# xmindflow/cenet

Hardware: AMD Instinct MI355X
Metric: training images/sec (224x224, 4-class) (higher is better)
Workload: dtype bf16

## Files before the change

cenet_amd/csrc/conv_direct.hip:

```cpp
#include "common.h"
#include "../../include/cenet_hip.h"

#define TH 8
#define TW 32
typedef bf16_t bf;

__device__ __forceinline__ unsigned cd_f2bf(float f) { return cenet_f2bf(f); }

struct ConvDirectArgs {
  const bf16_t* x;
  const float* w;
  bf16_t* y;
  int B, H, W, dgrad, tiles_x, tiles_y, ntiles;
};

template <int CIN, int COUT, int KS, int NW>
__global__ __launch_bounds__(64 * NW, (CIN == 64 && COUT == 64) ? 1 : 2) void conv_direct_bf16_kernel(ConvDirectArgs a) {
  constexpr int NT = 64 * NW, RPW = TH / NW, NI = 2 * RPW;
  constexpr int CQ = CIN / 8, HH = TH + KS - 1, HW_ = TW + KS - 1, KK = KS * KS, PADK = KS / 2;
  constexpr int UNITS = CQ * HH * HW_;
  constexpr int UPT = (UNITS + NT - 1) / NT;
  constexpr int MT = COUT / 16;
  __shared__ __attribute__((aligned(16))) bf Ws[KK * CQ * COUT * 8];
  __shared__ __attribute__((aligned(16))) bf Xs[UNITS * 8];
  const int tid = threadIdx.x, wave = tid >> 6, lane = tid & 63, fr = lane & 15, fq = lane >> 4;

  for (int e = tid; e < KK * CIN * COUT; e += NT) {
    const int t = e % KK, rest = e / KK;
    int co, ci;
    float v;
    if (!a.dgrad) {
      ci = rest % CIN;
      co = rest / CIN;
      v = a.w[e];
    } else {
      co = rest % COUT;
      ci = rest / COUT;
      v = a.w[(long)(ci * COUT + co) * KK + (KK - 1 - t)];
    }
    Ws[((t * CQ + (ci >> 3)) * COUT + co) * 8 + (ci & 7)] = (bf)cd_f2bf(v);
// ... 30 lines not shown
      const int s = tid + NT * u;
      if (s < UNITS) {
        unsigned pk[4];
#pragma unroll
        for (int j = 0; j < 4; ++j) pk[j] = pre[u][2 * j] | (pre[u][2 * j + 1] << 16);
        memcpy(&Xs[s * 8], pk, 16);
      }
    }
  };

  const int G = gridDim.x < 8 ? (int)gridDim.x : 8;
  const int xcd = blockIdx.x % G, nloc = ((int)gridDim.x + G - 1 - xcd) / G;
  const int per = (a.ntiles + G - 1) / G;
  const int t_end = (xcd + 1) * per < a.ntiles ? (xcd + 1) * per : a.ntiles;
  int tile = xcd * per + (int)blockIdx.x / G;
  if (tile < t_end) load_halo(tile);
  for (; tile < t_end; tile += nloc) {
    __syncthreads();
    store_halo();
    __syncthreads();
    const int nxt = tile + nloc;
    if (nxt < t_end) load_halo(nxt);

    f32x4 acc[MT][NI];
#pragma unroll
    for (int mi = 0; mi < MT; ++mi)
#pragma unroll
      for (int ni = 0; ni < NI; ++ni) acc[mi][ni] = f32x4{0.f, 0.f, 0.f, 0.f};
#pragma unroll
    for (int t = 0; t < KK; ++t) {
// ... 5 lines not shown
#pragma unroll
        for (int mi = 0; mi < MT; ++mi) memcpy(&wf[mi], &Ws[((t * CQ + kb * 4 + fq) * COUT + mi * 16 + fr) * 8], 16);
#pragma unroll
        for (int ni = 0; ni < NI; ++ni) {
          const int row = RPW * wave + (ni >> 1), xs = 16 * (ni & 1);
          bf16x8 xf;
          memcpy(&xf, &Xs[(((kb * 4 + fq) * HH + row + ky) * HW_ + xs + fr + kx) * 8], 16);
#pragma unroll
          for (int mi = 0; mi < MT; ++mi) acc[mi][ni] = __builtin_amdgcn_mfma_f32_16x16x32_bf16(xf, wf[mi], acc[mi][ni], 0, 0, 0);
        }
      }
    }
    const int b = tile / (a.tiles_x * a.tiles_y), tt = tile - b * (a.tiles_x * a.tiles_y);
    const int ty = tt / a.tiles_x, tx = tt - ty * a.tiles_x;
    bf16_t* yb = a.y + (long)b * COUT * HWp;
#pragma unroll
    for (int ni = 0; ni < NI; ++ni) {
      const int oy = ty * TH + RPW * wave + (ni >> 1), ox = tx * TW + 16 * (ni & 1) + 4 * fq;
      if (oy < a.H && ox < a.W) {
#pragma unroll
        for (int mi = 0; mi < MT; ++mi) {
          bf16_t* dst = yb + (long)(mi * 16 + fr) * HWp + (long)oy * a.W + ox;
          if (ox + 3 < a.W && (a.W & 3) == 0) {
            float v[4] = {acc[mi][ni][0], acc[mi][ni][1], acc[mi][ni][2], acc[mi][ni][3]};
            st4v(dst, v);
          } else {
#pragma unroll
            for (int r = 0; r < 4; ++r)
              if (ox + r < a.W) stf(dst + r, acc[mi][ni][r]);
          }
        }
      }
    }
  }
}

extern "C" int cenet_conv_direct_supported(int Cin, int Cout, int k, int stride, int pad) {
  if (stride != 1 || pad != k / 2) return 0;
  if (k == 5 && Cin == 32 && Cout == 32) return 1;
  if (k == 3 && Cin == 64 && (Cout == 64 || Cout == 32)) return 1;
  if (k == 3 && Cin == 32 && Cout == 64) return 1;
  return 0;
}

extern "C" int cenet_conv_direct_bf16(const bf16_t* x, const float* w, bf16_t* y, int B, int Cin, int Cout, int H, int W, int k,
                                      int dgrad, hipStream_t stream) {
  if (!x || !w || !y || B <= 0 || H <= 0 || W <= 0) return CENET_EINVAL;
  if (((uintptr_t)y & 7) != 0) return CENET_EINVAL;
  if (!cenet_conv_direct_supported(Cin, Cout, k, 1, k / 2)) return CENET_EUNSUPPORTED;
  ConvDirectArgs a;
  a.x = x; a.w = w; a.y = y; a.B = B; a.H = H; a.W = W; a.dgrad = dgrad;
  a.tiles_x = cdiv(W, TW);
  a.tiles_y = cdiv(H, TH);
  a.ntiles = B * a.tiles_x * a.tiles_y;
  const bool two = !(k == 3 && Cin == 64 && Cout == 64);
  const int slots = two ? 512 : 256;
  int grid = a.ntiles < slots ? a.ntiles : slots;
  if (k == 5 && Cin == 32 && Cout == 32) {
    CENET_LAUNCH((conv_direct_bf16_kernel<32, 32, 5, 4>), dim3(grid), dim3(256), stream, a);
  } else if (k == 3 && Cin == 64 && Cout == 64) {
    CENET_LAUNCH((conv_direct_bf16_kernel<64, 64, 3, 8>), dim3(grid), dim3(512), stream, a);
  } else if (k == 3 && Cin == 64 && Cout == 32) {
    CENET_LAUNCH((conv_direct_bf16_kernel<64, 32, 3, 8>), dim3(grid), dim3(512), stream, a);
  } else {
    CENET_LAUNCH((conv_direct_bf16_kernel<32, 64, 3, 4>), dim3(grid), dim3(256), stream, a);
  }
  CENET_CHECK_LAUNCH();
  return CENET_OK;
}

struct ConvWgradArgs {
  const bf16_t* x;
  const bf16_t* dy;
  float* ws;
  int B, H, W, tiles_x, tiles_y, ntiles;
  int vec;
};

__device__ __forceinline__ unsigned funnel16(unsigned lo, unsigned hi) { return (lo >> 16) | (hi << 16); }

template <int V>
// ... 264 lines not shown
```

cenet_amd/csrc/norm.hip:

```cpp
#include "common.h"
#include <cstdlib>
#include "../../include/cenet_hip.h"

template <typename T>
__global__ __launch_bounds__(256) void layernorm_fwd_kernel(const T* __restrict__ x, const float* __restrict__ gamma,
                                                           const float* __restrict__ beta, T* __restrict__ y,
                                                           float* __restrict__ mean, float* __restrict__ rstd, int rows,
                                                           int C, float eps) {
  const int wave = threadIdx.x >> 6, lane = threadIdx.x & 63;
  const long row = (long)blockIdx.x * 4 + wave;
  if (row >= rows) return;
  const T* xr = x + row * C;
  float s = 0.f;
  for (int c = lane; c < C; c += 64) s += ldf(xr + c);
  const float mu = wave_sum(s) / C;
  float v = 0.f;
  for (int c = lane; c < C; c += 64) {
    float d = ldf(xr + c) - mu;
    v += d * d;
  }
  const float rs = rsqrtf(wave_sum(v) / C + eps);
  T* yr = y + row * C;
  for (int c = lane; c < C; c += 64) stf(yr + c, (ldf(xr + c) - mu) * rs * gamma[c] + beta[c]);
  if (lane == 0) {
// ... 1381 lines not shown
  BnFin fin;
  fin.S = bn_partial_launch<T>(x, sxb, B, C, HW, ws, stream);
  fin.ws = ws; fin.n = (float)((long)B * HW); fin.mean = mean; fin.var = var; fin.rmean = running_mean; fin.rvar = running_var;
  fin.momentum = momentum; fin.nbt = num_batches_tracked; fin.nbt_n = nbt_count;
  return bn_apply_launch<T>(x, sxb, y, syb, mean, var, eps, gamma, beta, act, slope, B, C, HW, fin, stream);
}
CENET_TWIN(bn_train_fwd, (const T* x, long sxb, T* y, long syb, float* ws, float* mean, float* var, float* running_mean,
                          float* running_var, float momentum, long* num_batches_tracked, float eps, const float* gamma,
                          const float* beta, int act, float slope, int B, int C, int HW, int nbt_count, hipStream_t stream),
           (x, sxb, y, syb, ws, mean, var, running_mean, running_var, momentum, num_batches_tracked, eps, gamma, beta, act, slope, B,
            C, HW, nbt_count, stream))
CENET_TWIN(bn_apply, (const T* x, long sxb, T* y, long syb, const float* mean, const float* var, float eps, const float* gamma,
                      const float* beta, int act, float slope, int B, int C, int HW, hipStream_t stream),
           (x, sxb, y, syb, mean, var, eps, gamma, beta, act, slope, B, C, HW, stream))

template <typename T>
static int bn_bwd_acc_impl(const T* dy, long sgb, const T* x, long sxb, T* dx, long sdb, const float* mean, const float* var,
                           float eps, const float* gamma, const float* beta, int act, float slope, int B, int C, int HW,
                           float* ws, float* dgamma_acc, float* dbeta_acc, hipStream_t stream, const T* dx_add = nullptr,
                           long sab = 0) {
  if (B <= 0 || C <= 0 || HW <= 0) return CENET_EINVAL;
  const long total = (long)B * HW;
  if (sizeof(T) == 2 && total <= 256 * BN1K_EPT) {
    CENET_LAUNCH(bn_bwd_1k_kernel, dim3(C), dim3(256), stream, (const bf16_t*)dy, sgb, (const bf16_t*)x, sxb, (bf16_t*)dx, sdb, mean,
                 var, eps, gamma, beta, act, slope, B, HW, dgamma_acc, dbeta_acc, (const bf16_t*)dx_add, sab);
    CENET_CHECK_LAUNCH();
    return CENET_OK;
  }
  if (bn_flat_ok<T>(C, HW, sgb, sxb, sdb) && (!dx_add || sab == (long)C * HW)) {
    const bool v4 = bn_v4_ok<T>(HW, dy, sgb, x, sxb, dx, sdb) && bn_v4_ok<T>(HW, dx_add, sab, x, sxb, dx, sdb);
// ... 57 lines not shown
```

cenet_amd/kern.py:

```python
from __future__ import annotations

import ctypes as C
import math
from typing import Optional

import torch

from . import _lib
from ._lib import EpiT, MatT

ACT = {"none": 0, "relu": 1, "lrelu": 2, "gelu": 3, "silu": 4, "sigmoid": 5}


def _chk(*ts):
    for t in ts:
        if t is None:
            continue
        if isinstance(t, Ptr):
            t = t.t
        if t.dtype not in (torch.float32, torch.bfloat16, torch.int32, torch.int64, torch.uint8):
            raise TypeError(f"cenet_amd kernels take fp32 / bf16 tensors (int32 / int64 / uint8 for indices and masks); "
                            f"got {t.dtype}")
        if not t.is_cuda and not _lib.is_hostsim():
            raise RuntimeError("cenet_amd kernels run on the MI355X only: tensor is not on a CUDA/HIP device "
# ... 1035 lines not shown
        _lib.check(_lib.lib().cenet_zero_bytes(P(t), L(nbytes), stream()), "cenet_zero_bytes")
    return t


def conv_direct_supported(Cin: int, Cout: int, k: int, stride: int, pad: int) -> bool:
    return bool(_lib.lib().cenet_conv_direct_supported(int(Cin), int(Cout), int(k), int(stride), int(pad)))


def conv_direct(x, w, y, B, Cin, Cout, H, W, k, dgrad):
    _chk(x, w, y)
    assert x.dtype == BF16 and y.dtype == BF16 and w.dtype == torch.float32
    rc = _lib.lib().cenet_conv_direct_bf16(P(x), P(w), P(y), B, Cin, Cout, H, W, k, int(dgrad), stream())
    _lib.check(rc, "cenet_conv_direct_bf16")


def conv_c1_supported(Cin: int, Cout: int, k: int, stride: int, pad: int) -> bool:
    return bool(_lib.lib().cenet_conv_c1_supported(int(Cin), int(Cout), int(k), int(stride), int(pad)))


def conv_c1_fwd(x, w, y, B, Cout, H, W, k):
    _chk(x, w, y)
    assert x.dtype == BF16 and y.dtype == BF16 and w.dtype == torch.float32
    _lib.check(_lib.lib().cenet_conv_c1_fwd_bf16(P(x), P(w), P(y), B, Cout, H, W, k, stream()), "cenet_conv_c1_fwd_bf16")


def conv_c1_wgrad(x, dy, dw, B, Cout, H, W, k):
    _chk(x, dy, dw)
    assert x.dtype == BF16 and dy.dtype == BF16 and dw.dtype == torch.float32
    _lib.check(_lib.lib().cenet_conv_c1_wgrad_bf16(P(x), P(dy), P(dw), B, Cout, H, W, k, stream()), "cenet_conv_c1_wgrad_bf16")

# ... 115 lines not shown
```

cenet_amd/networks/cenet/modules/blocks.py:

```python
from __future__ import annotations

import math

import torch.nn as nn

from .... import ops


def bn_call(bn: nn.BatchNorm2d, x, act="none", slope=0.0, tap=False):
    return ops.batchnorm(x, bn.weight, bn.bias, bn.running_mean, bn.running_var, bn.num_batches_tracked, bn.training,
                         bn.eps, act, slope, ops.bn_momentum(bn), tap)


def _init_conv(m, scheme="normal"):
    if isinstance(m, nn.Conv2d):
        if scheme == "normal":
            nn.init.normal_(m.weight, std=.02)
        else:
            fan_out = m.kernel_size[0] * m.kernel_size[1] * m.out_channels // m.groups
            nn.init.normal_(m.weight, 0, math.sqrt(2.0 / fan_out))
        if m.bias is not None:
            nn.init.zeros_(m.bias)
    elif isinstance(m, nn.BatchNorm2d):
        nn.init.ones_(m.weight)
        nn.init.zeros_(m.bias)

# ... 52 lines not shown

    def __init__(self, in_channels, out_channels, kernel_size=3, stride=1, activation='relu'):
        super().__init__()
        if stride != 1 or activation != "leakyrelu":
            raise NotImplementedError("CENet uses UpConv(stride=1, leakyrelu) only")
        self.kernel_size = kernel_size
        self.up = nn.Sequential(
            nn.Upsample(scale_factor=2, mode='bilinear', align_corners=True),
            nn.Conv2d(in_channels, out_channels, kernel_size, stride=1, padding=kernel_size // 2, bias=False),
            nn.BatchNorm2d(out_channels),
            nn.LeakyReLU(0.2))
        self.apply(_init_conv)

    def forward(self, x):
        x = ops.interpolate_bilinear(x, scale_factor=2, align_corners=True)
        x = ops.conv2d_nchw(x, self.up[1].weight, None, stride=1, pad=self.kernel_size // 2)
        return bn_call(self.up[2], x, "lrelu", 0.2)
```

cenet_amd/networks/cenet/modules/unet.py:

```python
from __future__ import annotations

import torch.nn as nn

from .... import ops
from .blocks import bn_call


def _conv_layer(cin, cout, k, bias=False):
    seq = nn.Sequential()
    seq.add_module("conv", nn.Conv2d(cin, cout, k, stride=1, padding=k // 2, bias=bias))
    return seq


def _init(m):
    if isinstance(m, (nn.Conv2d, nn.Linear)):
        nn.init.trunc_normal_(m.weight, std=0.02)
        if m.bias is not None:
            nn.init.zeros_(m.bias)


class UnetResBlock(nn.Module):
    def __init__(self, spatial_dims, in_channels, out_channels, kernel_size, stride, norm_name,
                 act_name=("leakyrelu", {"inplace": True, "negative_slope": 0.01}), dropout=None):
        super().__init__()
# ... 2 lines not shown
        self.k = kernel_size
        self.slope = act_name[1].get("negative_slope", 0.01)
        self.conv1 = _conv_layer(in_channels, out_channels, kernel_size)
        self.conv2 = _conv_layer(out_channels, out_channels, kernel_size)
        self.lrelu = nn.LeakyReLU(self.slope)
        self.norm1 = nn.BatchNorm2d(out_channels)
        self.norm2 = nn.BatchNorm2d(out_channels)
        self.downsample = in_channels != out_channels
        if self.downsample:
            self.conv3 = _conv_layer(in_channels, out_channels, 1)
            self.norm3 = nn.BatchNorm2d(out_channels)
        self.apply(_init)

    def forward(self, inp, pool_scale=None):
        p = self.k // 2
        out = ops.conv2d_nchw(inp, self.conv1.conv.weight, None, stride=1, pad=p)
        out = bn_call(self.norm1, out, "lrelu", self.slope)
        out = ops.conv2d_nchw(out, self.conv2.conv.weight, None, stride=1, pad=p)
        if pool_scale is not None and self.downsample:
            if ops.res_tail_img_pool_supported(out, inp, self.conv3.conv.weight, self.norm2, self.norm3, pool_scale):
                return ops.res_tail_img_pool(out, self.norm2, inp, self.conv3.conv.weight, self.norm3, pool_scale, self.slope)
            res = ops.conv1x1(inp, self.conv3.conv.weight)
            if ops.res_tail_pool_supported(out, res, self.norm2, self.norm3, pool_scale):
                return ops.res_tail_pool(out, self.norm2, res, self.norm3, pool_scale, self.slope)
            y = ops.add_act(bn_call(self.norm2, out), bn_call(self.norm3, res), "lrelu", self.slope)
            return ops.maxpool2_scale(y, pool_scale)
        out = bn_call(self.norm2, out)
        res = inp
        if self.downsample:
            res = bn_call(self.norm3, ops.conv1x1(inp, self.conv3.conv.weight))
        y = ops.add_act(out, res, "lrelu", self.slope)
        return ops.maxpool2_scale(y, pool_scale) if pool_scale is not None else y

# ... 10 lines not shown
```

cenet_amd/ops/decoder_fused.py:

```python
from __future__ import annotations

import contextlib
import math
import os
from typing import Optional, Sequence

import torch
from torch.autograd import Function

from .. import kern
from .infra import *
from .linear import *
from .norm import *
from .depthwise import *
from .attention import *
from .glue import *


class BilinearFn(Function):

    @staticmethod
    def forward(ctx, x, Ho, Wo, sh, sw, align, tap=False):
        x = _c(x)
        B, Cn, Hi, Wi = x.shape
# ... 350 lines not shown
        x, w = ctx.saved_tensors
        g = _c(g)
        B, Cn, Hi, Wi = x.shape
        dx = torch.empty_like(x)
        kern.maxpool2_bwd(x, g, Cn * (Hi // 2) * (Wi // 2), dx, w, grad_buf(ctx.refs[0]), B, Cn, Hi, Wi)
        return dx, None


def maxpool2_scale(x, w):
    return MaxPool2ScaleFn.apply(x, w)


class ResTailPoolFn(Function):

    @staticmethod
    def forward(ctx, x2, x3, w, slope, g2, b2, rm2, rv2, nbt2, eps2, mom2, g3, b3, rm3, rv3, nbt3, eps3, mom3):
        x2, x3 = _c(x2), _c(x3)
        B, Cn, H, Wd = x2.shape
        HW = H * Wd
        st = []
        for x, rm, rv, nbt, mom in ((x2, rm2, rv2, nbt2, mom2), (x3, rm3, rv3, nbt3, mom3)):
            mean, var = _empty((Cn,), x), _empty((Cn,), x)
            ws = _empty((2 * Cn * 256,), x)
            kern.bn_stats(x, Cn * HW, B, Cn, HW, ws, mean, var, rm, rv, mom, nbt)
            st += [mean, var]
        wv = _c(w.reshape(-1))
        out = _act((B, Cn, H // 2, Wd // 2), x2)
        kern.res_tail_fwd(x2, x3, st[0], st[1], g2, b2, eps2, st[2], st[3], g3, b3, eps3, wv, slope, out, B, Cn, H, Wd)
        ctx.save_for_backward(x2, x3, wv, g2, b2, g3, b3, *st)
        ctx.refs = (w, g2, b2, g3, b3)
        ctx.cfg = (slope, eps2, eps3)
        return out

    @staticmethod
    def backward(ctx, g):
        x2, x3, wv, g2, b2, g3, b3, m2, v2, m3, v3 = ctx.saved_tensors
        wp, g2p, b2p, g3p, b3p = ctx.refs
        slope, eps2, eps3 = ctx.cfg
        g = _c(g)
        B, Cn, H, Wd = x2.shape
        dx2, dx3 = torch.empty_like(x2), torch.empty_like(x3)
        dw = grad_buf(wp)
        kern.res_tail_bwd(g, x2, x3, m2, v2, g2, b2, eps2, m3, v3, g3, b3, eps3, wv, slope, dx2, dx3, grad_buf(g2p), grad_buf(b2p),
                          grad_buf(g3p), grad_buf(b3p), dw.view(-1) if dw is not None else None, B, Cn, H, Wd)
        return (dx2, dx3) + (None,) * 16


def res_tail_pool(x2, bn2, x3, bn3, w, slope):
    return ResTailPoolFn.apply(x2, x3, w, slope, bn2.weight, bn2.bias, bn2.running_mean, bn2.running_var, bn2.num_batches_tracked,
                               bn2.eps, bn_momentum(bn2), bn3.weight, bn3.bias, bn3.running_mean,
                               bn3.running_var, bn3.num_batches_tracked, bn3.eps, bn_momentum(bn3))


class ResTailImgPoolFn(Function):
    _dummy: dict = {}

    @staticmethod
    def forward(ctx, x2, img, w3, w, slope, g2, b2, rm2, rv2, nbt2, eps2, mom2, g3, b3, rm3, rv3, nbt3, eps3, mom3):
        x2, img = _c(x2), _c(img)
        B, Cn, H, Wd = x2.shape
        HW = H * Wd
        mean2, var2 = _empty((Cn,), x2), _empty((Cn,), x2)
        kern.bn_stats(x2, Cn * HW, B, Cn, HW, _empty((2 * Cn * 256,), x2), mean2, var2, rm2, rv2, mom2, nbt2)
        key = (x2.device.type, x2.device.index)
        dm = ResTailImgPoolFn._dummy.get(key)
        if dm is None:
            dm = ResTailImgPoolFn._dummy[key] = (torch.zeros(1, device=x2.device), torch.ones(1, device=x2.device),
                                                 torch.zeros(1, device=x2.device, dtype=torch.long))
        imean, ivar = _empty((1,), x2), _empty((1,), x2)
        kern.bn_stats(img, HW, B, 1, HW, _empty((2 * 256,), x2), imean, ivar, dm[0], dm[1], 0.0, dm[2])
        wv, w3v = _c(w.reshape(-1)), _c(w3.reshape(-1))
        out = _act((B, Cn, H // 2, Wd // 2), x2)
        kern.res_tail_img_fwd(x2, img, mean2, var2, g2, b2, eps2, imean, ivar, w3v, g3, b3, eps3, rm3, rv3, nbt3, mom3, wv, slope, out,
                              B, Cn, H, Wd)
        ctx.save_for_backward(x2, img, wv, w3v, g2, b2, g3, b3, mean2, var2, imean, ivar)
        ctx.refs = (w, w3, g2, b2, g3, b3)
        ctx.cfg = (slope, eps2, eps3)
        return out

    @staticmethod
    def backward(ctx, g):
        x2, img, wv, w3v, g2, b2, g3, b3, mean2, var2, imean, ivar = ctx.saved_tensors
        wp, w3p, g2p, b2p, g3p, b3p = ctx.refs
        slope, eps2, eps3 = ctx.cfg
        g = _c(g)
        B, Cn, H, Wd = x2.shape
        dx2 = torch.empty_like(x2)
        dw, dw3 = grad_buf(wp), grad_buf(w3p)
        kern.res_tail_img_bwd(g, x2, img, mean2, var2, g2, b2, eps2, imean, ivar, w3v, g3, b3, eps3, wv, slope, dx2, grad_buf(g2p),
                              grad_buf(b2p), grad_buf(g3p), grad_buf(b3p), dw3.view(-1) if dw3 is not None else None,
                              dw.view(-1) if dw is not None else None, B, Cn, H, Wd)
        return (dx2,) + (None,) * 18


def res_tail_img_pool(x2, bn2, img, w3, bn3, w, slope):
    return ResTailImgPoolFn.apply(x2, img, w3, w, slope, bn2.weight, bn2.bias, bn2.running_mean, bn2.running_var,
                                  bn2.num_batches_tracked, bn2.eps, bn_momentum(bn2), bn3.weight,
                                  bn3.bias, bn3.running_mean, bn3.running_var, bn3.num_batches_tracked, bn3.eps,
                                  bn_momentum(bn3))


def res_tail_img_pool_supported(x2, img, w3, bn2, bn3, w) -> bool:
    return bool(bn2.training and bn3.training and _bf(x2) and _bf(img) and img.dim() == 4 and img.shape[1] == 1
                and not img.requires_grad and tuple(w3.shape[1:]) == (1, 1, 1) and w3.shape[0] == x2.shape[1]
                and img.shape[0] == x2.shape[0] and tuple(img.shape[2:]) == tuple(x2.shape[2:]) and w.numel() == x2.shape[1]
                and x2.data_ptr() % 16 == 0 and img.data_ptr() % 16 == 0
                and kern._lib.lib().cenet_res_tail_supported(int(x2.shape[2]), int(x2.shape[3]))
                and os.environ.get("CENET_RES_TAIL_FUSED", "1") not in ("0", "x3"))


def res_tail_pool_supported(x2, x3, bn2, bn3, w) -> bool:
    return bool(bn2.training and bn3.training and x2.is_cuda == x3.is_cuda and kern.res_tail_supported(x2, x3)
                and w.numel() == x2.shape[1] and os.environ.get("CENET_RES_TAIL_FUSED", "1") != "0")

# ... 3 lines not shown
```

cenet_amd/ops/linear.py:

```python
from __future__ import annotations

import contextlib
import math
import os
from typing import Optional, Sequence

import torch
from torch.autograd import Function

from .. import kern
from .infra import *


class LinearFn(Function):

    @staticmethod
    def forward(ctx, x, W, b, resid, bscale, split_k=False, tap=False):
        x = _c(x)
        K = x.shape[-1]
        N = W.shape[0]
        R = x.numel() // K
        M = R
        bs_rows = 0 if bscale is None else R // x.shape[0]
        resid = _c(resid)
# ... 204 lines not shown
            else:
                kern.gemm(kern.mat_plain(kern.wq(Wp, x), 1, Cin, kfast=0), kern.mat_plain(g, HW, 1, sb=Cout * HW), dx, Cin, HW,
                          Cout, scr=HW, scc=1, scb=Cin * HW, nbatch=B, R=g_tap, srb=Cin * HW, srr=HW, src=1)
        elif g_tap is not None:
            dx = g_tap
        return dx, None, None, (g if ctx.has_resid else None), None


def conv1x1(x, W, b=None, resid=None, tap=False):
    return Conv1x1Fn.apply(x, W, b, resid, tap)


class Conv2dFn(Function):

    @staticmethod
    def forward(ctx, x, W, b, geom):
        B, Cin, H, Wd, sb, sc, sy, sx, stride, pad, out_layout = geom
        Cout, _, k, _ = W.shape
        Ho = (H + 2 * pad - k) // stride + 1
        Wo = (Wd + 2 * pad - k) // stride + 1
        Kd = Cin * k * k
        plain_nchw = (sb == Cin * H * Wd and sc == H * Wd and sy == Wd and sx == 1 and out_layout == "nchw" and b is None)
        ctx.direct = bool(plain_nchw and _bf(x) and kern.conv_direct_supported(Cin, Cout, k, stride, pad))
        ctx.c1 = bool(plain_nchw and _bf(x) and not ctx.direct and kern.conv_c1_supported(Cin, Cout, k, stride, pad))
        if ctx.c1:
            y = _act((B, Cout, Ho, Wo), x)
            kern.conv_c1_fwd(x, W, y, B, Cout, H, Wd, k)
            ctx.save_for_backward(x, W)
            ctx.refs = (W, b)
            ctx.geom = geom
            ctx.out_hw = (Ho, Wo)
            return y
        if ctx.direct:
            y = _act((B, Cout, Ho, Wo), x)
            kern.conv_direct(x, W, y, B, Cin, Cout, H, Wd, k, 0)
            ctx.save_for_backward(x, W)
            ctx.refs = (W, b)
            ctx.geom = geom
            ctx.out_hw = (Ho, Wo)
            return y
        Bm = kern.mat_im2col(x, sb=sb, skb=0, sci=sc, sy=sy, sx=sx, KH=k, KW=k, Pw=Wo, Hs=H, Ws=Wd, stride=stride,
                             pad=pad, dil=1, patch_is_row=1, transposed=0, kfast=0)
        shape = (B, Cout, Ho, Wo) if out_layout == "nchw" else (B, Ho * Wo, Cout)
        scr, scc = (Ho * Wo, 1) if out_layout == "nchw" else (1, Cout)
        tiles = B * ((Cout + 63) // 64) * ((Ho * Wo + 63) // 64)
        Wq = kern.wq(W, x)
        if tiles <= 256 and Kd >= 1024 and _bf(x):
            if b is None:
                y = _zeros(shape, x)
            else:
# ... 61 lines not shown
                    kern.conv_c1_wgrad(x, g, dW, B, Cout, H, Wd, k)
                elif (dW is not None and getattr(ctx, "direct", False) and _bf(g)
                        and kern.conv_wgrad_direct_supported(Cin, Cout, k, stride, pad)):
                    kern.conv_wgrad_direct(x, g, dW, B, Cin, Cout, H, Wd, k)
                elif dW is not None:
                    Bm = kern.mat_im2col(x, sb=0, skb=sb, sci=sc, sy=sy, sx=sx, KH=k, KW=k, Pw=Wo, Hs=H, Ws=Wd, stride=stride,
                                         pad=pad, dil=1, patch_is_row=0, transposed=0, kfast=1)
                    iters = B * ((Ho * Wo + 31) // 32)
                    kern.gemm(kern.mat_plain(g, g_sc, g_sp, skb=Cout * Ho * Wo, kfast=int(g_sp == 1)), Bm, dW, Cout, Kd,
                              Ho * Wo, scr=Kd, scc=1, nkb=B, splits=kern.pick_splits(Cout, Kd, 1, iters), atomic=True)
                if db is not None:
                    if out_layout == "nchw":
                        kern.chan_dot(g, Cout * Ho * Wo, None, 0, db, B, Cout, Ho * Wo)
                    else:
                        kern.col_sum(g, db, B * Ho * Wo, Cout)
        return dx, (dW if derived else None), None, None


class ChanSumWeightFn(Function):

    @staticmethod
    def forward(ctx, W):
        ctx.ref = W
        return W.sum(1, keepdim=True)

    @staticmethod
    def backward(ctx, g):
        dW = grad_buf(ctx.ref)
        if dW is not None:
            dW.add_(g)
        return None


def chan_sum_weight(W):
    return ChanSumWeightFn.apply(W)


def conv2d_nchw(x, W, b=None, stride=1, pad=0, out_layout="nchw", expand_channels: int = 0):
    x = _c(x)
    B, C, H, Wd = x.shape
    if expand_channels and C == 1:
        geom = (B, expand_channels, H, Wd, H * Wd, 0, Wd, 1, stride, pad, out_layout)
    else:
        geom = (B, C, H, Wd, C * H * Wd, H * Wd, Wd, 1, stride, pad, out_layout)
    return Conv2dFn.apply(x, W, b, geom)


class PatchTokFn(Function):

    @staticmethod
    def forward(ctx, x, H, Wd, s):
        x = _c(x)
        B, N, C = x.shape
        Ho, Wo = H // s, Wd // s
        xp = _act((B, Ho * Wo, C * s * s), x)
        kern.patch_tok(x, xp, B, Ho, Wo, C, s)
        ctx.geom = (B, Ho, Wo, C, s, N)
        return xp

    @staticmethod
# ... 44 lines not shown
```

cenet_amd/ops/norm.py:

```python
from __future__ import annotations

import contextlib
import math
import os
from typing import Optional, Sequence

import torch
from torch.autograd import Function

from .. import kern
from .infra import *
from .linear import *


class LayerNormFn(Function):
    @staticmethod
    def forward(ctx, x, gamma, beta, eps, up_scale=None):
        ctx.up_scale = up_scale
        x = _c(x)
        Cn = x.shape[-1]
        rows = x.numel() // Cn
        y = torch.empty_like(x)
        mean, rstd = _empty((rows,), x), _empty((rows,), x)
        kern.layernorm_fwd(x, gamma, beta, y, mean, rstd, rows, Cn, eps)
# ... 113 lines not shown
        dx = torch.empty_like(x)
        dg, db = grad_buf(gp), grad_buf(bp)
        if dg is None:
            dg, db = _zeros((Cn,), x), _zeros((Cn,), x)
        _ln_bwd(g, x, gamma, mean, rstd, dx, dg, db, rows, Cn, dx_add=_c(g_res), up_scale=ctx.up_scale)
        return dx, None, None, None, None


def layernorm_res(x, gamma, beta, eps):
    return LayerNormResFn.apply(x, gamma, beta, eps, getattr(x, "_cenet_bscale", None))


class BatchNormFn(Function):

    @staticmethod
    def forward(ctx, x, weight, bias, rmean, rvar, nbt, training, eps, act, slope, momentum, tap=False):
        x = _c(x)
        B, Cn = x.shape[:2]
        HW = x.numel() // (B * Cn)
        y = torch.empty_like(x)
        if training:
            mean, var = _empty((Cn,), x), _empty((Cn,), x)
            ws = _empty((2 * Cn * 256,), x)
            kern.bn_train_fwd(x, Cn * HW, y, Cn * HW, ws, mean, var, rmean, rvar, momentum, nbt, eps, weight, bias, act, slope,
                              B, Cn, HW)
        else:
            mean, var = rmean, rvar
            kern.bn_apply(x, Cn * HW, y, Cn * HW, mean, var, eps, weight, bias, act, slope, B, Cn, HW)
        ctx.save_for_backward(x, weight, bias, mean, var)
        ctx.refs = (weight, bias)
        ctx.cfg = (training, eps, act, slope)
        return (y, x.view_as(x)) if tap else y

    @staticmethod
    def backward(ctx, g, g_tap=None):
        x, weight, bias, mean, var = ctx.saved_tensors
        wp, bp = ctx.refs
        training, eps, act, slope = ctx.cfg
        if g is None:
            return (g_tap,) + (None,) * 11
        if not training:
            raise RuntimeError("cenet_amd BatchNorm backward is implemented for training mode only")
        g = _c(g)
        if g_tap is not None:
            g_tap = _c(g_tap) if g_tap.dtype == g.dtype else _c(g_tap.to(g.dtype))
        B, Cn = x.shape[:2]
        HW = x.numel() // (B * Cn)
        dx = torch.empty_like(x)
        ws = _empty((2 * Cn * 256,), x)
        dg, db = grad_buf(wp), grad_buf(bp)
        if dg is None:
            dg, db = _zeros((Cn,), x), _zeros((Cn,), x)
        kern.bn_bwd(g, Cn * HW, x, Cn * HW, dx, Cn * HW, mean, var, eps, weight, bias, act, slope, B, Cn, HW, ws, dg, db,
                    dx_add=g_tap)
        return (dx,) + (None,) * 11


def batchnorm(x, weight, bias, rmean, rvar, nbt, training, eps=1e-5, act="none", slope=0.0, momentum=0.1, tap=False):
    return BatchNormFn.apply(x, weight, bias, rmean, rvar, nbt, training, eps, act, slope, momentum, tap)


__all__ = [n for n in dir() if not n.startswith("__")]
```

include/cenet_hip.h:

```cpp
#ifndef CENET_HIP_H
#define CENET_HIP_H

#ifdef __cplusplus
extern "C" {
#endif

#ifndef CENET_HOSTSIM_BUILD
typedef struct ihipStream_t* cenet_stream_t;
#else
typedef void* cenet_stream_t;
#endif

typedef struct {
  const void* ptr;
  long sb, sb2, skb, sr, sc;
  long sk_outer;
  int kinner;
  int mode, kfast;
  int patch_is_row, transposed;
  int KH, KW, Pw, Hs, Ws, stride, pad, dil;
  long sci, sy, sx;
} cenet_mat_t;

typedef struct {
// ... 25 lines not shown
  const void* B;
  float* C;
  float* asum;
  long lda, ldb, skbA, skbB;
  int M, N, K, nkb;
  int akf, bkf;
} cenet_wgrad_prob_t;
long cenet_wgrad_group_ws_floats(const cenet_wgrad_prob_t* p, int n);
int cenet_wgrad_group_bf16(const cenet_wgrad_prob_t* p, int n, float* ws, long ws_floats, cenet_stream_t stream);
int cenet_wgrad_group_plan(const cenet_wgrad_prob_t* p, int n, int* launch, int* bm, int* bn, int* ns);
int cenet_wgrad_group_phase_bf16(const cenet_wgrad_prob_t* p, int n, float* ws, long ws_floats, int phase, cenet_stream_t stream);

int cenet_conv_direct_supported(int Cin, int Cout, int k, int stride, int pad);
int cenet_conv_direct_bf16(const unsigned short* x, const float* w, unsigned short* y, int B, int Cin, int Cout, int H, int W,
                           int k, int dgrad, cenet_stream_t stream);
int cenet_conv_c1_supported(int Cin, int Cout, int k, int stride, int pad);
int cenet_pw_fewout_supported(int Cin, int Cout);
int cenet_pw_fewout_wgrad_supported(int Cin, int Cout);
int cenet_pw_fewout_fwd_bf16(const unsigned short* x, const unsigned short* W, const float* bias, unsigned short* y, int B, int Cin,
    int Cout, long HW, cenet_stream_t stream);
int cenet_pw_fewout_dgrad_bf16(const unsigned short* dy, const unsigned short* W, unsigned short* dx, int B, int Cin, int Cout,
    long HW, cenet_stream_t stream);
int cenet_pw_fewout_wgrad_bf16(const unsigned short* x, const unsigned short* dy, float* dW_acc, float* dbias_acc, int B, int Cin,
    int Cout, long HW, cenet_stream_t stream);
int cenet_pw_small_supported(int G);
int cenet_pw_small_bf16(const unsigned short* x, const unsigned short* W, unsigned short* y, int B, int groups, int G, long HW,
    int transpose, cenet_stream_t stream);
int cenet_conv_c1_fwd_bf16(const unsigned short* x, const float* w, unsigned short* y, int B, int Cout, int H, int W, int k,
    cenet_stream_t stream);
int cenet_conv_c1_wgrad_bf16(const unsigned short* x, const unsigned short* dy, float* dw_acc, int B, int Cout, int H, int W,
// ... 560 lines not shown
```

Baseline: 1845.

## Fuse BatchNorm statistics into direct conv epilogue and skip separate stats pass

Adds a stats-producing variant of the direct conv kernel. It accumulates per-channel shifted sums and sums of squares of the bf16-rounded outputs in its epilogue, and writes per-block partials that a small finalize kernel merges into mean, var and running stats. The following BatchNorm then runs only the apply pass using those stats, which removes one full read of the conv output per BN in conv+BN blocks and in the res-tail fused paths. In exchange the conv epilogue gets more register pressure and an extra reduction, a finalize launch is added, and the feature is on by default behind an environment flag.

```diff
diff --git a/cenet_amd/csrc/conv_direct.hip b/cenet_amd/csrc/conv_direct.hip
--- a/cenet_amd/csrc/conv_direct.hip
+++ b/cenet_amd/csrc/conv_direct.hip
@@ -12,10 +12,11 @@
   const float* w;
   bf16_t* y;
   int B, H, W, dgrad, tiles_x, tiles_y, ntiles;
+  float* stats;
 };
 
-template <int CIN, int COUT, int KS, int NW>
-__global__ __launch_bounds__(64 * NW, (CIN == 64 && COUT == 64) ? 1 : 2) void conv_direct_bf16_kernel(ConvDirectArgs a) {
+template <int CIN, int COUT, int KS, int NW, bool ST>
+__device__ __forceinline__ void conv_direct_body(const ConvDirectArgs& a) {
   constexpr int NT = 64 * NW, RPW = TH / NW, NI = 2 * RPW;
   constexpr int CQ = CIN / 8, HH = TH + KS - 1, HW_ = TW + KS - 1, KK = KS * KS, PADK = KS / 2;
   constexpr int UNITS = CQ * HH * HW_;
@@ -23,7 +24,11 @@
   constexpr int MT = COUT / 16;
   __shared__ __attribute__((aligned(16))) bf Ws[KK * CQ * COUT * 8];
   __shared__ __attribute__((aligned(16))) bf Xs[UNITS * 8];
+  __shared__ float sshift[ST ? COUT : 1];
   const int tid = threadIdx.x, wave = tid >> 6, lane = tid & 63, fr = lane & 15, fq = lane >> 4;
+  float shift[MT], s1[MT], s2[MT], cnt = 0.f;
+#pragma unroll
+  for (int mi = 0; mi < MT; ++mi) shift[mi] = s1[mi] = s2[mi] = 0.f;
 
   for (int e = tid; e < KK * CIN * COUT; e += NT) {
     const int t = e % KK, rest = e / KK;
@@ -84,6 +89,7 @@
   const int per = (a.ntiles + G - 1) / G;
   const int t_end = (xcd + 1) * per < a.ntiles ? (xcd + 1) * per : a.ntiles;
   int tile = xcd * per + (int)blockIdx.x / G;
+  const int tile0 = tile;
   if (tile < t_end) load_halo(tile);
   for (; tile < t_end; tile += nloc) {
     __syncthreads();
@@ -119,24 +125,133 @@
     const int b = tile / (a.tiles_x * a.tiles_y), tt = tile - b * (a.tiles_x * a.tiles_y);
     const int ty = tt / a.tiles_x, tx = tt - ty * a.tiles_x;
     bf16_t* yb = a.y + (long)b * COUT * HWp;
+    if (ST && tile == tile0) {
+      if (wave == 0 && fq == 0) {
+#pragma unroll
+        for (int mi = 0; mi < MT; ++mi) sshift[mi * 16 + fr] = cenet_bf2f(cd_f2bf(acc[mi][0][0]));
+      }
+      __syncthreads();
+#pragma unroll
+      for (int mi = 0; mi < MT; ++mi) shift[mi] = sshift[mi * 16 + fr];
+    }
 #pragma unroll
     for (int ni = 0; ni < NI; ++ni) {
       const int oy = ty * TH + RPW * wave + (ni >> 1), ox = tx * TW + 16 * (ni & 1) + 4 * fq;
       if (oy < a.H && ox < a.W) {
+        const bool full = ox + 3 < a.W && (a.W & 3) == 0;
+        if (ST) cnt += (float)(a.W - ox < 4 ? a.W - ox : 4);
 #pragma unroll
         for (int mi = 0; mi < MT; ++mi) {
           bf16_t* dst = yb + (long)(mi * 16 + fr) * HWp + (long)oy * a.W + ox;
-          if (ox + 3 < a.W && (a.W & 3) == 0) {
-            float v[4] = {acc[mi][ni][0], acc[mi][ni][1], acc[mi][ni][2], acc[mi][ni][3]};
-            st4v(dst, v);
+          if (!ST) {
+            if (full) {
+              float v[4] = {acc[mi][ni][0], acc[mi][ni][1], acc[mi][ni][2], acc[mi][ni][3]};
+              st4v(dst, v);
+            } else {
+#pragma unroll
+              for (int r = 0; r < 4; ++r)
+                if (ox + r < a.W) stf(dst + r, acc[mi][ni][r]);
+            }
           } else {
-#pragma unroll
-            for (int r = 0; r < 4; ++r)
-              if (ox + r < a.W) stf(dst + r, acc[mi][ni][r]);
+            const unsigned u[2] = {cenet_pack_bf2(acc[mi][ni][0], acc[mi][ni][1]), cenet_pack_bf2(acc[mi][ni][2], acc[mi][ni][3])};
+            if (full) {
+              memcpy(dst, u, 8);
+            } else {
+#pragma unroll
+              for (int r = 0; r < 4; ++r)
+                if (ox + r < a.W) dst[r] = (bf16_t)((u[r >> 1] >> (16 * (r & 1))) & 0xFFFFu);
+            }
+#pragma unroll
+            for (int r = 0; r < 4; ++r) {
+              const float d = cenet_bf2f((u[r >> 1] >> (16 * (r & 1))) & 0xFFFFu) - shift[mi];
+              if (full || ox + r < a.W) {
+                s1[mi] += d;
+                s2[mi] += d * d;
+              }
+            }
           }
         }
       }
     }
+  }
+  if (ST) {
+    float* red = reinterpret_cast<float*>(Xs);
+    static_assert(NW * 3 * COUT * 4 <= UNITS * 16, "the fold fits the halo tile");
+    cnt += __shfl_xor(cnt, 16);
+    cnt += __shfl_xor(cnt, 32);
+#pragma unroll
+    for (int mi = 0; mi < MT; ++mi) {
+      s1[mi] += __shfl_xor(s1[mi], 16);
+      s1[mi] += __shfl_xor(s1[mi], 32);
+      s2[mi] += __shfl_xor(s2[mi], 16);
+      s2[mi] += __shfl_xor(s2[mi], 32);
+    }
+    __syncthreads();
+    if (fq == 0) {
+#pragma unroll
+      for (int mi = 0; mi < MT; ++mi) {
+        red[(wave * 3 + 0) * COUT + mi * 16 + fr] = cnt;
+        red[(wave * 3 + 1) * COUT + mi * 16 + fr] = s1[mi];
+        red[(wave * 3 + 2) * COUT + mi * 16 + fr] = s2[mi];
+      }
+    }
+    __syncthreads();
+    if (tid < COUT) {
+      float n = 0.f, t1 = 0.f, t2 = 0.f;
+#pragma unroll
+      for (int w = 0; w < NW; ++w) {
+        n += red[(w * 3 + 0) * COUT + tid];
+        t1 += red[(w * 3 + 1) * COUT + tid];
+        t2 += red[(w * 3 + 2) * COUT + tid];
+      }
+      float* row = a.stats + (long)blockIdx.x * 3 * COUT;
+      const bool any = tile0 < t_end;
+      const float m = any ? t1 / n : 0.f;
+      row[tid] = any ? n : 0.f;
+      row[COUT + tid] = any ? sshift[tid] + m : 0.f;
+      row[2 * COUT + tid] = any ? fmaxf(t2 - t1 * m, 0.f) : 0.f;
+    }
+  }
+}
+
+template <int CIN, int COUT, int KS, int NW>
+__global__ __launch_bounds__(64 * NW, (CIN == 64 && COUT == 64) ? 1 : 2) void conv_direct_bf16_kernel(ConvDirectArgs a) {
+  conv_direct_body<CIN, COUT, KS, NW, false>(a);
+}
+template <int CIN, int COUT, int KS, int NW>
+__global__ __launch_bounds__(64 * NW, (CIN == 64 && COUT == 64) ? 1 : 2) void conv_direct_stats_bf16_kernel(ConvDirectArgs a) {
+  conv_direct_body<CIN, COUT, KS, NW, true>(a);
+}
+
+__global__ __launch_bounds__(64) void conv_stats_finalize_kernel(const float* __restrict__ rows, int R, int C, float* __restrict__ mean,
+                                                                 float* __restrict__ var, float* running_mean, float* running_var,
+                                                                 float momentum, long* nbt) {
+  const int c = blockIdx.x, lane = threadIdx.x;
+  const float m0 = rows[C + c];
+  float sa = 0.f, sn = 0.f;
+  for (int i = lane; i < R; i += 64) {
+    const float n = rows[(long)i * 3 * C + c];
+    sa += n * (rows[((long)i * 3 + 1) * C + c] - m0);
+    sn += n;
+  }
+  sa = wave_sum(sa);
+  sn = wave_sum(sn);
+  const float mu = m0 + sa / sn;
+  float q = 0.f;
+  for (int i = lane; i < R; i += 64) {
+    const float n = rows[(long)i * 3 * C + c], d = rows[((long)i * 3 + 1) * C + c] - mu;
+    q += rows[((long)i * 3 + 2) * C + c] + n * d * d;
+  }
+  q = wave_sum(q);
+  if (lane == 0) {
+    const float v = fmaxf(q / sn, 0.f);
+    mean[c] = mu;
+    var[c] = v;
+    if (running_mean) {
+      running_mean[c] = (1.f - momentum) * running_mean[c] + momentum * mu;
+      running_var[c] = (1.f - momentum) * running_var[c] + momentum * v * (sn / (sn - 1.f));
+    }
+    if (nbt && c == 0) nbt[0] += 1;
   }
 }
 
@@ -154,7 +269,7 @@
   if (((uintptr_t)y & 7) != 0) return CENET_EINVAL;
   if (!cenet_conv_direct_supported(Cin, Cout, k, 1, k / 2)) return CENET_EUNSUPPORTED;
   ConvDirectArgs a;
-  a.x = x; a.w = w; a.y = y; a.B = B; a.H = H; a.W = W; a.dgrad = dgrad;
+  a.x = x; a.w = w; a.y = y; a.B = B; a.H = H; a.W = W; a.dgrad = dgrad; a.stats = nullptr;
   a.tiles_x = cdiv(W, TW);
   a.tiles_y = cdiv(H, TH);
   a.ntiles = B * a.tiles_x * a.tiles_y;
@@ -170,6 +285,38 @@
   } else {
     CENET_LAUNCH((conv_direct_bf16_kernel<32, 64, 3, 4>), dim3(grid), dim3(256), stream, a);
   }
+  CENET_CHECK_LAUNCH();
+  return CENET_OK;
+}
+
+#define CENET_CD_MAX_GRID 512
+extern "C" int cenet_conv_direct_stats_supported(int Cin, int Cout, int k, int stride, int pad) {
+  if (stride != 1 || pad != k / 2) return 0;
+  return (k == 5 && Cin == 32 && Cout == 32) || (k == 3 && Cin == 64 && (Cout == 64 || Cout == 32));
+}
+extern "C" long cenet_conv_direct_stats_ws_floats(int Cout) { return 3L * CENET_CD_MAX_GRID * Cout; }
+extern "C" int cenet_conv_direct_stats_bf16(const bf16_t* x, const float* w, bf16_t* y, int B, int Cin, int Cout, int H, int W, int k,
+                                            float* ws, float* mean, float* var, float* running_mean, float* running_var,
+                                            float momentum, long* num_batches_tracked, hipStream_t stream) {
+  if (!x || !w || !y || !ws || !mean || !var || B <= 0 || H <= 0 || W <= 0) return CENET_EINVAL;
+  if (((uintptr_t)y & 7) != 0 || (long)B * H * W < 2) return CENET_EINVAL;
+  if (!cenet_conv_direct_stats_supported(Cin, Cout, k, 1, k / 2)) return CENET_EUNSUPPORTED;
+  ConvDirectArgs a;
+  a.x = x; a.w = w; a.y = y; a.B = B; a.H = H; a.W = W; a.dgrad = 0; a.stats = ws;
+  a.tiles_x = cdiv(W, TW);
+  a.tiles_y = cdiv(H, TH);
+  a.ntiles = B * a.tiles_x * a.tiles_y;
+  const int slots = (k == 3 && Cout == 64) ? 256 : CENET_CD_MAX_GRID;
+  const int grid = a.ntiles < slots ? a.ntiles : slots;
+  if (k == 5) {
+    CENET_LAUNCH((conv_direct_stats_bf16_kernel<32, 32, 5, 4>), dim3(grid), dim3(256), stream, a);
+  } else if (Cout == 64) {
+    CENET_LAUNCH((conv_direct_stats_bf16_kernel<64, 64, 3, 8>), dim3(grid), dim3(512), stream, a);
+  } else {
+    CENET_LAUNCH((conv_direct_stats_bf16_kernel<64, 32, 3, 8>), dim3(grid), dim3(512), stream, a);
+  }
+  CENET_LAUNCH(conv_stats_finalize_kernel, dim3(Cout), dim3(64), stream, (const float*)ws, grid, Cout, mean, var, running_mean,
+               running_var, momentum, num_batches_tracked);
   CENET_CHECK_LAUNCH();
   return CENET_OK;
 }
diff --git a/cenet_amd/csrc/norm.hip b/cenet_amd/csrc/norm.hip
--- a/cenet_amd/csrc/norm.hip
+++ b/cenet_amd/csrc/norm.hip
@@ -1419,6 +1419,13 @@
                       const float* beta, int act, float slope, int B, int C, int HW, hipStream_t stream),
            (x, sxb, y, syb, mean, var, eps, gamma, beta, act, slope, B, C, HW, stream))
 
+extern "C" int cenet_bn_fold_apply_bf16(const bf16_t* x, long sxb, bf16_t* y, long syb, const float* mean, const float* var, float eps,
+                                        const float* gamma, const float* beta, int act, float slope, int B, int C, int HW,
+                                        hipStream_t stream) {
+  if (!x || !y || !mean || !var || !gamma || !beta) return CENET_EINVAL;
+  return bn_apply_impl<bf16_t>(x, sxb, y, syb, mean, var, eps, gamma, beta, act, slope, B, C, HW, stream);
+}
+
 template <typename T>
 static int bn_bwd_acc_impl(const T* dy, long sgb, const T* x, long sxb, T* dx, long sdb, const float* mean, const float* var,
                            float eps, const float* gamma, const float* beta, int act, float slope, int B, int C, int HW,
diff --git a/cenet_amd/kern.py b/cenet_amd/kern.py
--- a/cenet_amd/kern.py
+++ b/cenet_amd/kern.py
@@ -2,6 +2,7 @@
 
 import ctypes as C
 import math
+import os
 from typing import Optional
 
 import torch
@@ -1073,6 +1074,31 @@
     _lib.check(rc, "cenet_conv_direct_bf16")
 
 
+def bn_fold_enabled() -> bool:
+    return os.environ.get("CENET_BN_FOLD", "1") != "0"
+
+
+def conv_direct_stats_supported(Cin: int, Cout: int, k: int, stride: int, pad: int) -> bool:
+    return bool(_lib.lib().cenet_conv_direct_stats_supported(int(Cin), int(Cout), int(k), int(stride), int(pad)))
+
+
+def conv_direct_stats(x, w, y, B, Cin, Cout, H, W, k, mean, var, rmean, rvar, momentum, nbt):
+    _chk(x, w, y, mean, var, rmean, rvar)
+    assert x.dtype == BF16 and y.dtype == BF16 and w.dtype == torch.float32
+    f = _lib.lib().cenet_conv_direct_stats_ws_floats
+    f.restype = C.c_long
+    ws = torch.empty(int(f(int(Cout))), device=x.device, dtype=torch.float32)
+    rc = _lib.lib().cenet_conv_direct_stats_bf16(P(x), P(w), P(y), B, Cin, Cout, H, W, k, P(ws), P(mean), P(var), P(rmean), P(rvar),
+                                                 C.c_float(momentum), P(nbt), stream())
+    _lib.check(rc, "cenet_conv_direct_stats_bf16")
+
+
+def bn_fold_apply(x, sxb, y, syb, mean, var, eps, gamma, beta, act, slope, B, Cn, HW):
+    _chk(x, y, mean, var, gamma, beta)
+    assert x.dtype == BF16 and y.dtype == BF16
+    _call("cenet_bn_fold_apply_bf16", x, L(sxb), y, L(syb), mean, var, float(eps), gamma, beta, ACT[act], float(slope), B, Cn, HW)
+
+
 def conv_c1_supported(Cin: int, Cout: int, k: int, stride: int, pad: int) -> bool:
     return bool(_lib.lib().cenet_conv_c1_supported(int(Cin), int(Cout), int(k), int(stride), int(pad)))
 
diff --git a/cenet_amd/networks/cenet/modules/blocks.py b/cenet_amd/networks/cenet/modules/blocks.py
--- a/cenet_amd/networks/cenet/modules/blocks.py
+++ b/cenet_amd/networks/cenet/modules/blocks.py
@@ -9,7 +9,7 @@
 
 def bn_call(bn: nn.BatchNorm2d, x, act="none", slope=0.0, tap=False):
     return ops.batchnorm(x, bn.weight, bn.bias, bn.running_mean, bn.running_var, bn.num_batches_tracked, bn.training,
-                         bn.eps, act, slope, ops.bn_momentum(bn), tap)
+                         bn.eps, act, slope, ops.bn_momentum(bn), tap, ops.pending_bn_stats(x, bn))
 
 
 def _init_conv(m, scheme="normal"):
@@ -92,5 +92,5 @@
 
     def forward(self, x):
         x = ops.interpolate_bilinear(x, scale_factor=2, align_corners=True)
-        x = ops.conv2d_nchw(x, self.up[1].weight, None, stride=1, pad=self.kernel_size // 2)
+        x = ops.conv2d_nchw(x, self.up[1].weight, None, stride=1, pad=self.kernel_size // 2, bn=self.up[2])
         return bn_call(self.up[2], x, "lrelu", 0.2)
diff --git a/cenet_amd/networks/cenet/modules/unet.py b/cenet_amd/networks/cenet/modules/unet.py
--- a/cenet_amd/networks/cenet/modules/unet.py
+++ b/cenet_amd/networks/cenet/modules/unet.py
@@ -40,9 +40,9 @@
 
     def forward(self, inp, pool_scale=None):
         p = self.k // 2
-        out = ops.conv2d_nchw(inp, self.conv1.conv.weight, None, stride=1, pad=p)
+        out = ops.conv2d_nchw(inp, self.conv1.conv.weight, None, stride=1, pad=p, bn=self.norm1)
         out = bn_call(self.norm1, out, "lrelu", self.slope)
-        out = ops.conv2d_nchw(out, self.conv2.conv.weight, None, stride=1, pad=p)
+        out = ops.conv2d_nchw(out, self.conv2.conv.weight, None, stride=1, pad=p, bn=self.norm2)
         if pool_scale is not None and self.downsample:
             if ops.res_tail_img_pool_supported(out, inp, self.conv3.conv.weight, self.norm2, self.norm3, pool_scale):
                 return ops.res_tail_img_pool(out, self.norm2, inp, self.conv3.conv.weight, self.norm3, pool_scale, self.slope)
diff --git a/cenet_amd/ops/decoder_fused.py b/cenet_amd/ops/decoder_fused.py
--- a/cenet_amd/ops/decoder_fused.py
+++ b/cenet_amd/ops/decoder_fused.py
@@ -388,12 +388,15 @@
 class ResTailPoolFn(Function):
 
     @staticmethod
-    def forward(ctx, x2, x3, w, slope, g2, b2, rm2, rv2, nbt2, eps2, mom2, g3, b3, rm3, rv3, nbt3, eps3, mom3):
+    def forward(ctx, x2, x3, w, slope, g2, b2, rm2, rv2, nbt2, eps2, mom2, g3, b3, rm3, rv3, nbt3, eps3, mom3, stats2=None):
         x2, x3 = _c(x2), _c(x3)
         B, Cn, H, Wd = x2.shape
         HW = H * Wd
         st = []
         for x, rm, rv, nbt, mom in ((x2, rm2, rv2, nbt2, mom2), (x3, rm3, rv3, nbt3, mom3)):
+            if x is x2 and stats2 is not None:
+                st += list(stats2)
+                continue
             mean, var = _empty((Cn,), x), _empty((Cn,), x)
             ws = _empty((2 * Cn * 256,), x)
             kern.bn_stats(x, Cn * HW, B, Cn, HW, ws, mean, var, rm, rv, mom, nbt)
@@ -417,25 +420,28 @@
         dw = grad_buf(wp)
         kern.res_tail_bwd(g, x2, x3, m2, v2, g2, b2, eps2, m3, v3, g3, b3, eps3, wv, slope, dx2, dx3, grad_buf(g2p), grad_buf(b2p),
                           grad_buf(g3p), grad_buf(b3p), dw.view(-1) if dw is not None else None, B, Cn, H, Wd)
-        return (dx2, dx3) + (None,) * 16
+        return (dx2, dx3) + (None,) * 17
 
 
 def res_tail_pool(x2, bn2, x3, bn3, w, slope):
     return ResTailPoolFn.apply(x2, x3, w, slope, bn2.weight, bn2.bias, bn2.running_mean, bn2.running_var, bn2.num_batches_tracked,
                                bn2.eps, bn_momentum(bn2), bn3.weight, bn3.bias, bn3.running_mean,
-                               bn3.running_var, bn3.num_batches_tracked, bn3.eps, bn_momentum(bn3))
+                               bn3.running_var, bn3.num_batches_tracked, bn3.eps, bn_momentum(bn3), pending_bn_stats(x2, bn2))
 
 
 class ResTailImgPoolFn(Function):
     _dummy: dict = {}
 
     @staticmethod
-    def forward(ctx, x2, img, w3, w, slope, g2, b2, rm2, rv2, nbt2, eps2, mom2, g3, b3, rm3, rv3, nbt3, eps3, mom3):
+    def forward(ctx, x2, img, w3, w, slope, g2, b2, rm2, rv2, nbt2, eps2, mom2, g3, b3, rm3, rv3, nbt3, eps3, mom3, stats2=None):
         x2, img = _c(x2), _c(img)
         B, Cn, H, Wd = x2.shape
         HW = H * Wd
-        mean2, var2 = _empty((Cn,), x2), _empty((Cn,), x2)
-        kern.bn_stats(x2, Cn * HW, B, Cn, HW, _empty((2 * Cn * 256,), x2), mean2, var2, rm2, rv2, mom2, nbt2)
+        if stats2 is not None:
+            mean2, var2 = stats2
+        else:
+            mean2, var2 = _empty((Cn,), x2), _empty((Cn,), x2)
+            kern.bn_stats(x2, Cn * HW, B, Cn, HW, _empty((2 * Cn * 256,), x2), mean2, var2, rm2, rv2, mom2, nbt2)
         key = (x2.device.type, x2.device.index)
         dm = ResTailImgPoolFn._dummy.get(key)
         if dm is None:
@@ -464,14 +470,14 @@
         kern.res_tail_img_bwd(g, x2, img, mean2, var2, g2, b2, eps2, imean, ivar, w3v, g3, b3, eps3, wv, slope, dx2, grad_buf(g2p),
                               grad_buf(b2p), grad_buf(g3p), grad_buf(b3p), dw3.view(-1) if dw3 is not None else None,
                               dw.view(-1) if dw is not None else None, B, Cn, H, Wd)
-        return (dx2,) + (None,) * 18
+        return (dx2,) + (None,) * 19
 
 
 def res_tail_img_pool(x2, bn2, img, w3, bn3, w, slope):
     return ResTailImgPoolFn.apply(x2, img, w3, w, slope, bn2.weight, bn2.bias, bn2.running_mean, bn2.running_var,
                                   bn2.num_batches_tracked, bn2.eps, bn_momentum(bn2), bn3.weight,
                                   bn3.bias, bn3.running_mean, bn3.running_var, bn3.num_batches_tracked, bn3.eps,
-                                  bn_momentum(bn3))
+                                  bn_momentum(bn3), pending_bn_stats(x2, bn2))
 
 
 def res_tail_img_pool_supported(x2, img, w3, bn2, bn3, w) -> bool:
diff --git a/cenet_amd/ops/linear.py b/cenet_amd/ops/linear.py
--- a/cenet_amd/ops/linear.py
+++ b/cenet_amd/ops/linear.py
@@ -242,7 +242,7 @@
 class Conv2dFn(Function):
 
     @staticmethod
-    def forward(ctx, x, W, b, geom):
+    def forward(ctx, x, W, b, geom, fold=None):
         B, Cin, H, Wd, sb, sc, sy, sx, stride, pad, out_layout = geom
         Cout, _, k, _ = W.shape
         Ho = (H + 2 * pad - k) // stride + 1
@@ -261,7 +261,13 @@
             return y
         if ctx.direct:
             y = _act((B, Cout, Ho, Wo), x)
-            kern.conv_direct(x, W, y, B, Cin, Cout, H, Wd, k, 0)
+            if fold is not None and kern.conv_direct_stats_supported(Cin, Cout, k, stride, pad) and B * H * Wd >= 2:
+                rm, rv, nbt, mom, holder = fold
+                mean, var = _empty((Cout,), x), _empty((Cout,), x)
+                kern.conv_direct_stats(x, W, y, B, Cin, Cout, H, Wd, k, mean, var, rm, rv, mom, nbt)
+                holder["stats"] = (mean, var)
+            else:
+                kern.conv_direct(x, W, y, B, Cin, Cout, H, Wd, k, 0)
             ctx.save_for_backward(x, W)
             ctx.refs = (W, b)
             ctx.geom = geom
@@ -353,7 +359,7 @@
                         kern.chan_dot(g, Cout * Ho * Wo, None, 0, db, B, Cout, Ho * Wo)
                     else:
                         kern.col_sum(g, db, B * Ho * Wo, Cout)
-        return dx, (dW if derived else None), None, None
+        return dx, (dW if derived else None), None, None, None
 
 
 class ChanSumWeightFn(Function):
@@ -375,14 +381,25 @@
     return ChanSumWeightFn.apply(W)
 
 
-def conv2d_nchw(x, W, b=None, stride=1, pad=0, out_layout="nchw", expand_channels: int = 0):
+def conv2d_nchw(x, W, b=None, stride=1, pad=0, out_layout="nchw", expand_channels: int = 0, bn=None):
     x = _c(x)
     B, C, H, Wd = x.shape
     if expand_channels and C == 1:
         geom = (B, expand_channels, H, Wd, H * Wd, 0, Wd, 1, stride, pad, out_layout)
     else:
         geom = (B, C, H, Wd, C * H * Wd, H * Wd, Wd, 1, stride, pad, out_layout)
+    if bn is not None and bn.training and _bf(x) and b is None and kern.bn_fold_enabled():
+        holder = {}
+        y = Conv2dFn.apply(x, W, b, geom, (bn.running_mean, bn.running_var, bn.num_batches_tracked, bn_momentum(bn), holder))
+        if "stats" in holder:
+            y._cenet_bn_stats = holder["stats"] + (bn,)
+        return y
     return Conv2dFn.apply(x, W, b, geom)
+
+
+def pending_bn_stats(x, bn):
+    st = getattr(x, "_cenet_bn_stats", None)
+    return st[:2] if st is not None and st[2] is bn and bn.training else None
 
 
 class PatchTokFn(Function):
diff --git a/cenet_amd/ops/norm.py b/cenet_amd/ops/norm.py
--- a/cenet_amd/ops/norm.py
+++ b/cenet_amd/ops/norm.py
@@ -151,12 +151,15 @@
 class BatchNormFn(Function):
 
     @staticmethod
-    def forward(ctx, x, weight, bias, rmean, rvar, nbt, training, eps, act, slope, momentum, tap=False):
+    def forward(ctx, x, weight, bias, rmean, rvar, nbt, training, eps, act, slope, momentum, tap=False, stats=None):
         x = _c(x)
         B, Cn = x.shape[:2]
         HW = x.numel() // (B * Cn)
         y = torch.empty_like(x)
-        if training:
+        if training and stats is not None:
+            mean, var = stats
+            kern.bn_fold_apply(x, Cn * HW, y, Cn * HW, mean, var, eps, weight, bias, act, slope, B, Cn, HW)
+        elif training:
             mean, var = _empty((Cn,), x), _empty((Cn,), x)
             ws = _empty((2 * Cn * 256,), x)
             kern.bn_train_fwd(x, Cn * HW, y, Cn * HW, ws, mean, var, rmean, rvar, momentum, nbt, eps, weight, bias, act, slope,
@@ -175,7 +178,7 @@
         wp, bp = ctx.refs
         training, eps, act, slope = ctx.cfg
         if g is None:
-            return (g_tap,) + (None,) * 11
+            return (g_tap,) + (None,) * 12
         if not training:
             raise RuntimeError("cenet_amd BatchNorm backward is implemented for training mode only")
         g = _c(g)
@@ -190,11 +193,11 @@
             dg, db = _zeros((Cn,), x), _zeros((Cn,), x)
         kern.bn_bwd(g, Cn * HW, x, Cn * HW, dx, Cn * HW, mean, var, eps, weight, bias, act, slope, B, Cn, HW, ws, dg, db,
                     dx_add=g_tap)
-        return (dx,) + (None,) * 11
-
-
-def batchnorm(x, weight, bias, rmean, rvar, nbt, training, eps=1e-5, act="none", slope=0.0, momentum=0.1, tap=False):
-    return BatchNormFn.apply(x, weight, bias, rmean, rvar, nbt, training, eps, act, slope, momentum, tap)
+        return (dx,) + (None,) * 12
+
+
+def batchnorm(x, weight, bias, rmean, rvar, nbt, training, eps=1e-5, act="none", slope=0.0, momentum=0.1, tap=False, stats=None):
+    return BatchNormFn.apply(x, weight, bias, rmean, rvar, nbt, training, eps, act, slope, momentum, tap, stats)
 
 
 __all__ = [n for n in dir() if not n.startswith("__")]
diff --git a/include/cenet_hip.h b/include/cenet_hip.h
--- a/include/cenet_hip.h
+++ b/include/cenet_hip.h
@@ -63,6 +63,14 @@
 int cenet_conv_direct_supported(int Cin, int Cout, int k, int stride, int pad);
 int cenet_conv_direct_bf16(const unsigned short* x, const float* w, unsigned short* y, int B, int Cin, int Cout, int H, int W,
                            int k, int dgrad, cenet_stream_t stream);
+int cenet_conv_direct_stats_supported(int Cin, int Cout, int k, int stride, int pad);
+long cenet_conv_direct_stats_ws_floats(int Cout);
+int cenet_conv_direct_stats_bf16(const unsigned short* x, const float* w, unsigned short* y, int B, int Cin, int Cout, int H, int W,
+                                 int k, float* ws, float* mean, float* var, float* running_mean, float* running_var, float momentum,
+                                 long* num_batches_tracked, cenet_stream_t stream);
+int cenet_bn_fold_apply_bf16(const unsigned short* x, long sxb, unsigned short* y, long syb, const float* mean, const float* var,
+                             float eps, const float* gamma, const float* beta, int act, float slope, int B, int C, int HW,
+                             cenet_stream_t stream);
 int cenet_conv_c1_supported(int Cin, int Cout, int k, int stride, int pad);
 int cenet_pw_fewout_supported(int Cin, int Cout);
 int cenet_pw_fewout_wgrad_supported(int Cin, int Cout);
```

Result: no change. 1844 (-0.0%).
